# npit/video-learning-tf

Hardware: AMD Instinct MI355X
Metric: clips/sec (16-frame 227x227) LRCN train step (higher is better)
Workload: dtype f32; 1 GPU; LRCN AlexNet(fc6)+LSTM(256) 16-frame 227x227x3 clips, 101 classes, UCF-101-shaped synthetic, full train step; global_batch=64, clips_per_gpu=64, frames_per_clip=16, parallelism=dp1, optimizer=sgd+clip_by_global_norm(10), init=reference (sigma 0.05), dist_world_size=1

## Files before the change

video-learning-tf_amd/csrc/mfma_gemm.hip:

```cpp
#include <stdlib.h>
#include <string.h>

#include "common.h"
#include "conv_desc.h"

typedef float f32x16 __attribute__((ext_vector_type(16)));
typedef const __attribute__((address_space(4))) int* const_int_ptr;
__device__ __forceinline__ const_int_ptr as_const(const int* p) { return (const_int_ptr)(uintptr_t)p; }
static constexpr int NT = 256;
static constexpr int KBLK = 16;

static constexpr uint32_t OOB_OFF = 0xF0000000u;
static constexpr int64_t MAX_BUF_BYTES = 0xE0000000ll;

__device__ __forceinline__ __amdgpu_buffer_rsrc_t make_rsrc(const float* base, int64_t bytes) {
    return __builtin_amdgcn_make_buffer_rsrc(const_cast<float*>(base), 0, (int)(uint32_t)bytes, 0x00020000);
}
__device__ __forceinline__ float buf_load(__amdgpu_buffer_rsrc_t r, uint32_t voff, int soff) {
    return __builtin_bit_cast(float, __builtin_amdgcn_raw_buffer_load_b32(r, (int)voff, soff, 0));
}

template <int BX, int BR>
struct LdsTile {
    static constexpr int STR = BR + 2;
// ... 799 lines not shown
            static_for<0, NMS>([&](auto MI) __attribute__((always_inline)) {
                constexpr int m = decltype(MI)::value;
                constexpr int prod = m / (TM * TN), a = (m % (TM * TN)) / TN, b = m % TN;
                acc[a][b] = mfma_bf16(As[c][a].p[kProdA[prod]], Bs[c][b].p[kProdB[prod]], acc[a][b]);
                constexpr int idx = st * NMS + m;
                static_for<0, FPM>([&](auto EI) __attribute__((always_inline)) {
                    constexpr int f = idx * FPM + decltype(EI)::value;
                    if constexpr (f < NF) {
                        if constexpr (X4) dma_x4(cur ^ 1, f, rt_next);
                        else dma(cur ^ 1, f, rt_next);
                    }
                });
                __builtin_amdgcn_sched_barrier(0x106);
                if constexpr (idx == LT) load_table(rt_next + 1);
                if constexpr (idx == PIN) {
                    int rtn = rt_next + 1;
                    asm volatile("" : "+s"(rtn));
                    decode(rtn);
                    pin_table();
                }
            });
        });
        finish_tile(cur ^ 1);
    };
    auto run_tile = [&](const int cur, int rt_next) __attribute__((always_inline)) {
        if constexpr (MATH != 0) tile_split(cur, rt_next);
        else tile(cur, rt_next);
    };
    int rt = rt0;
    for (int i = 0; i + 1 < ntiles; i += 2, rt += 2) {
        run_tile(0, rt + 1);
        run_tile(1, rt + 2);
    }
    if (ntiles > 0 && (ntiles & 1)) run_tile(0, rt + 1);

    EpiRowMajor::template apply<TM, TN>(pe, zg, zs, i0 + wi0, j0 + wj0, acc);
    if (ones_row >= 0) {
        float* dbs = db_slabs + (int64_t)zs * db_stride + zg * d.Cog;
        const int lr = ones_row - wi0;
        if (lr >= 0 && lr < BM / WM) {
            const int a = lr >> 5, rr = lr & 31;
            const int q = (rr & 3) + 4 * (rr >> 3);
            if (((rr >> 2) & 1) == (lane >> 5)) {
#pragma unroll
                for (int b = 0; b < TN; ++b) {
                    const int j = j0 + wj0 + 32 * b + (lane & 31);
                    float v = 0.f;
#pragma unroll
                    for (int aa = 0; aa < TM; ++aa)
#pragma unroll
                        for (int qq = 0; qq < 16; ++qq)
                            if (aa == a && qq == q) v = acc[aa][b][qq];
                    if (j < d.Cog) dbs[j] = v;
                }
            }
        }
    }
}

typedef float f32x4 __attribute__((ext_vector_type(4)));
typedef float f32x4u __attribute__((ext_vector_type(4), aligned(4)));

struct ConvDmaParams {
    const float* w;
    int64_t w_ld;
    int64_t w_grp_stride;
    int64_t w_bytes;
    const int* row_tab;
    int nblk;
};

struct ConvRowClasses {
    int ncls;
    int wg0[6];
    int S[5];
    int oh0[5], RW[5];
    FastDiv dRW[5];
    int K[5], tab0[5], rt0[5];
};

struct ConvTile {
    int bid;
    int S, oh0, RW;
    FastDiv dRW;
    int K, nblk;
    const int* ktab;
    const int* row_tab;
};

__device__ __forceinline__ ConvTile conv_pick_tile(const ConvRowClasses& rc, const ConvGeom& g, const ConvDmaParams& pa) {
    const int id = blockIdx.x;
    int w0 = 0, w1 = rc.wg0[1], S = rc.S[0], oh0 = rc.oh0[0], RW = rc.RW[0], K = rc.K[0], tab0 = rc.tab0[0], rt0 = rc.rt0[0];
    FastDiv dRW = rc.dRW[0];
#pragma unroll
    for (int c = 1; c < 5; ++c) {
        if (c < rc.ncls && id >= rc.wg0[c]) {
            w0 = rc.wg0[c]; w1 = rc.wg0[c + 1]; S = rc.S[c]; oh0 = rc.oh0[c]; RW = rc.RW[c]; K = rc.K[c]; tab0 = rc.tab0[c]; rt0 = rc.rt0[c];
            dRW = rc.dRW[c];
        }
    }
    ConvTile t;
    t.bid = xcd_swizzle(id - w0, w1 - w0);
    t.S = S; t.oh0 = oh0; t.RW = RW; t.dRW = dRW; t.K = K; t.nblk = (K + KBLK - 1) / KBLK;
    t.ktab = g.ktab + tab0;
    t.row_tab = pa.row_tab + rt0;
    return t;
}

struct ConvPixel {
    uint32_t n, p, oh, ow;
};
__device__ __forceinline__ ConvPixel conv_tile_pixel(const ConvTile& t, uint32_t m, const FastDiv& dOW, int OW) {
    ConvPixel q;
    q.n = fd_div(m, t.dRW);
    q.p = m - q.n * t.RW;
    const uint32_t r = fd_div(q.p, dOW);
    q.ow = q.p - r * OW;
    q.oh = r + t.oh0;
    return q;
}

template <int BM>
__device__ __forceinline__ uint32_t conv_weight_voff(int i0, int cl, int Cog) {
    return (cl < BM && i0 + cl < Cog) ? (uint32_t)(i0 + cl) * 4u : OOB_OFF;
}
__device__ __forceinline__ uint32_t conv_pixel_voff(const ConvTile& tl, const ConvGeom& g, int m) {
    const bool vm = m < tl.S;
    const ConvPixel q = conv_tile_pixel(tl, vm ? m : 0, g.dOW, g.OW);
    const int ih0 = (int)q.oh * g.stride - g.pt + g.halo, iw0 = (int)q.ow * g.col_mul + g.col_add;
    return vm ? (uint32_t)((int64_t)q.n * g.img_stride + (int64_t)ih0 * g.Wp + iw0) * 4u : OOB_OFF;
}

template <int SR>
struct ConvStageTab {
    int tabv[SR / 4];
    int row0 = 0;
    bool blk_ok = false;
    __device__ __forceinline__ void load(const ConvTile& tl, const ConvGeom& g, int wrow, int st) {
        const int k0 = st * SR + wrow;
        const const_int_ptr tt = as_const(tl.ktab) + k0 + st * g.zero;
#pragma unroll
        for (int f = 0; f < SR / 4; ++f) tabv[f] = tt[f];
        row0 = as_const(tl.row_tab)[k0 / KBLK + st * g.zero] + k0 % KBLK;
        blk_ok = k0 / KBLK < tl.nblk;
    }
    __device__ __forceinline__ void pin() {
#pragma unroll
        for (int f = 0; f < SR / 4; ++f) asm volatile("" : "+s"(tabv[f]));
        asm volatile("" : "+s"(row0));
    }
};

template <int SR>
__global__ __launch_bounds__(NT, 64 / SR) void conv_dma_kernel(const ConvDmaParams pa, const ConvGeom g, const EpiConvNCHW::Params pe, const ConvRowClasses rc,
                                                               int tiles_i, int wide) {
    constexpr int BM = 128, BN = 128;
    constexpr int ABUF = SR * BM, BUF = SR * (BM + BN);
    constexpr int RW = SR / 4;
    constexpr int NF = RW * 4;
    constexpr int NT2 = SR / 4;
    constexpr int FPM = 1;
    static_assert(SR == 64 || SR == 32, "stage depth");
    extern __shared__ __attribute__((aligned(16))) float ldsc[];
    const ConvTile tl = conv_pick_tile(rc, g, pa);
    const int ti_blk = tl.bid % tiles_i, tj_blk = tl.bid / tiles_i;
    const int zg = blockIdx.y;
    const int i0 = ti_blk * BM, j0 = tj_blk * BN;
    const int lane = threadIdx.x & 63;
    const int wave = __builtin_amdgcn_readfirstlane(threadIdx.x >> 6);
    const int wm = wave >> 1, wn = wave & 1;

    const i32x4 rs_w = rsrc_words(pa.w + (int64_t)zg * pa.w_grp_stride, pa.w_bytes - (int64_t)zg * pa.w_grp_stride * 4);
    const i32x4 rs_x = rsrc_words(g.x + (int64_t)zg * g.grp_stride, (g.total - (int64_t)zg * g.grp_stride) * 4);
    uint32_t voff_a[2], voff_b[2];
#pragma unroll
    for (int hf = 0; hf < 2; ++hf) {
        voff_a[hf] = conv_weight_voff<BM>(i0, hf * 64 + lane, pe.Cog);
        voff_b[hf] = conv_pixel_voff(tl, g, j0 + hf * 64 + lane);
    }
    const uint32_t lds0 = (uint32_t)(uintptr_t)(__attribute__((address_space(3))) float*)ldsc;
    const int ld_bytes = (int)(pa.w_ld * 4);

    ConvStageTab<SR> tab;
    int (&tabv)[RW] = tab.tabv;
    int& row0 = tab.row0;
    bool& blk_ok = tab.blk_ok;
    const int wrow = wave * RW;
    auto load_table = [&](int st) { tab.load(tl, g, wrow, st); };
    auto pin_table = [&]() { tab.pin(); };
    auto dma = [&](const int nb, const int f, int st) {
        const int rr = f >> 2, kind = f & 3, hf = kind & 1;
        const int z = st * g.zero;
        const uint32_t row_lds = lds0 + (uint32_t)(nb * BUF + (wrow + rr) * 128 + hf * 64 + z) * 4u;
        const bool live = blk_ok && st * SR + wrow + rr < tl.K;
        if (kind < 2) lds_dma_row(rs_w, row_lds, voff_a[hf], min(row0 + rr, g.K - 1) * ld_bytes);
        else lds_dma_row(rs_x, row_lds + ABUF * 4u, live ? voff_b[hf] : OOB_OFF, tabv[rr]);
    };
    int a_soff = 0;
    auto dma_fast = [&](const int nb, const int f, int st) {
        const int rr = f >> 2, kind = f & 3, hf = kind & 1;
        const uint32_t row_lds = lds0 + (uint32_t)(nb * BUF + (wrow + rr) * 128 + hf * 64 + st * g.zero) * 4u;
        if (f == 0) a_soff = row0 * ld_bytes;
        if (kind < 2) lds_dma_row(rs_w, row_lds, voff_a[hf], a_soff);
        else lds_dma_row(rs_x, row_lds + ABUF * 4u, voff_b[hf], tabv[rr]);
        if (kind == 1) a_soff += ld_bytes;
    };
    auto finish_stage = [&]() {
        asm volatile("s_waitcnt vmcnt(0)" ::: "memory");
        __syncthreads();
    };

    f32x16 acc[2][2];
#pragma unroll
    for (int a = 0; a < 2; ++a)
#pragma unroll
        for (int b = 0; b < 2; ++b)
#pragma unroll
            for (int q = 0; q < 16; ++q) acc[a][b][q] = 0.f;

    const int nstages = (tl.nblk * KBLK + SR - 1) / SR;
    load_table(0);
    pin_table();
#pragma unroll
    for (int f = 0; f < NF; ++f) dma(0, f, 0);
    load_table(1);
    pin_table();
    finish_stage();

    float bias_r[2][16];
#pragma unroll
    for (int a = 0; a < 2; ++a)
#pragma unroll
        for (int q = 0; q < 16; ++q) {
            const int co = i0 + wm * 64 + 2 * ((q & 3) + 8 * (q >> 2) + 4 * (lane >> 5)) + a;
            bias_r[a][q] = (pe.bias && co < pe.Cog) ? pe.bias[zg * pe.Cog + co] : 0.f;
        }

    const float* fa = ldsc + (lane >> 5) * 128 + wm * 64 + 2 * (lane & 31);
    const float* fb = ldsc + ABUF + (lane >> 5) * 128 + wn * 64 + (lane & 31);

    auto stage = [&](const int cur, const bool fast, int st_next) {
        float2 af[2], bf[2], an[2], bn[2];
        auto read_b = [&](int step) {
            const float* q = fb + cur * BUF + step * 256;
            return float2{q[0], q[32]};
        };
        af[0] = *reinterpret_cast<const float2*>(fa + cur * BUF);
        bf[0] = read_b(0);
        af[1] = *reinterpret_cast<const float2*>(fa + cur * BUF + 256);
        bf[1] = read_b(1);
#pragma unroll
        for (int t = 0; t < NT2; ++t) {
            if (t + 1 < NT2) {
#pragma unroll
                for (int u = 0; u < 2; ++u) {
                    an[u] = *reinterpret_cast<const float2*>(fa + cur * BUF + (2 * (t + 1) + u) * 256);
                    bn[u] = read_b(2 * (t + 1) + u);
                }
            }
#pragma unroll
            for (int m = 0; m < 8; ++m) {
                const int u = m >> 2, a = (m >> 1) & 1, b = m & 1;
                acc[a][b] = __builtin_amdgcn_mfma_f32_32x32x2f32(a ? af[u].y : af[u].x, b ? bf[u].y : bf[u].x, acc[a][b], 0, 0, 0);
                const int f = (t * 8 + m) * FPM;
                if (f < NF) {
#pragma unroll
                    for (int e = 0; e < FPM; ++e) {
                        if (fast) dma_fast(cur ^ 1, f + e, st_next);
                        else dma(cur ^ 1, f + e, st_next);
                    }
                    __builtin_amdgcn_sched_barrier(0);
                }
            }
            static_assert(NF / FPM / 8 <= NT2 - 4, "fetches must end before the table is replaced");
            if (t == NT2 - 4) {
                load_table(st_next + 1);
                __builtin_amdgcn_sched_barrier(0);
            }
            if (t == NT2 - 2) {
                pin_table();
                __builtin_amdgcn_sched_barrier(0);
            }
#pragma unroll
            for (int u = 0; u < 2; ++u) {
                af[u] = an[u];
                bf[u] = bn[u];
            }
        }
        finish_stage();
    };
    const int nfull = tl.K / SR;
    int st = 0;
    for (; st + 2 < nfull; st += 2) {
        stage(0, true, st + 1);
        stage(1, true, st + 2);
    }
    for (; st < nstages; ++st) {
        if (st & 1) stage(1, false, st + 1);
        else stage(0, false, st + 1);
    }

    if (wide) {
        constexpr int SP = BN + 4;
        float* T = ldsc;
#pragma unroll
        for (int b = 0; b < 2; ++b)
#pragma unroll
            for (int a = 0; a < 2; ++a)
#pragma unroll
                for (int q = 0; q < 16; ++q) {
                    const int i = (q & 3) + 8 * (q >> 2) + 4 * (lane >> 5);
                    float v = acc[a][b][q] + bias_r[a][q];
                    if (pe.relu) v = fmaxf(v, 0.f);
                    T[(wm * 64 + 2 * i + a) * SP + wn * 64 + 32 * b + (lane & 31)] = v;
                }
        __syncthreads();
        const int px = 4 * (lane & 31);
        const int m = j0 + px;
        const uint32_t n = fd_div((uint32_t)min(m, tl.S - 1), tl.dRW);
        const int p = m - (int)n * tl.RW;
        const bool run4 = m + 3 < tl.S && p + 3 < tl.RW;
        const int64_t cbase = ((int64_t)n * pe.Cout_total + (int64_t)zg * pe.Cog) * pe.y_plane + tl.oh0 * pe.OW + p;
#pragma unroll
        for (int i = 0; i < BM / 8; ++i) {
            const int cl = wave * (BM / 4) + 2 * i + (lane >> 5);
            const int co = i0 + cl;
            const f32x4 v = *reinterpret_cast<const f32x4*>(T + cl * SP + px);
            if (co >= pe.Cog) continue;
            float* dst = pe.y + cbase + (int64_t)co * pe.y_plane;
            if (run4) {
                *reinterpret_cast<f32x4u*>(dst) = v;
            } else {
#pragma unroll
                for (int e = 0; e < 4; ++e) {
                    const int me = m + e;
                    if (me < tl.S) {
                        const uint32_t ne = fd_div((uint32_t)me, tl.dRW);
                        const int pe_ = me - (int)ne * tl.RW + tl.oh0 * pe.OW;
                        pe.y[((int64_t)ne * pe.Cout_total + (int64_t)zg * pe.Cog + co) * pe.y_plane + pe_] = v[e];
                    }
                }
            }
        }
        return;
    }
#pragma unroll
    for (int b = 0; b < 2; ++b) {
        const int m = j0 + wn * 64 + 32 * b + (lane & 31);
        if (m >= tl.S) continue;
        const ConvPixel px = conv_tile_pixel(tl, m, pe.dOW, pe.OW);
        const int64_t c0 = (int64_t)px.n * pe.Cout_total + (int64_t)zg * pe.Cog;
        const int64_t ybase = c0 * pe.y_plane + (int64_t)(px.oh + pe.y_halo) * pe.y_wp + px.ow + pe.y_halo;
        const int64_t mbase = c0 * pe.m_plane + (int64_t)(px.oh + pe.m_halo) * pe.m_wp + px.ow + pe.m_halo;
#pragma unroll
        for (int a = 0; a < 2; ++a) {
            float mk[16];
            if (pe.mask) {
#pragma unroll
                for (int q = 0; q < 16; ++q) {
                    const int co = i0 + wm * 64 + 2 * ((q & 3) + 8 * (q >> 2) + 4 * (lane >> 5)) + a;
                    mk[q] = co < pe.Cog ? pe.mask[mbase + (int64_t)co * pe.m_plane] : 0.f;
                }
            }
#pragma unroll
            for (int q = 0; q < 16; ++q) {
                const int i = (q & 3) + 8 * (q >> 2) + 4 * (lane >> 5);
                const int co = i0 + wm * 64 + 2 * i + a;
                if (co < pe.Cog) {
                    float v = acc[a][b][q] + bias_r[a][q];
                    if (pe.relu) v = fmaxf(v, 0.f);
                    if (pe.mask) v = mk[q] > 0.f ? v : 0.f;
                    pe.y[ybase + (int64_t)co * pe.y_plane] = v;
                }
            }
        }
    }
}


__global__ void conv_wsplit_kernel(const float* __restrict__ w, int64_t w_ld, int64_t w_grp_stride, const int* __restrict__ row_tab,
                                   int K, int Cog, int CogP, int nstages, int planes, uint32_t* __restrict__ out) {
    const int st = blockIdx.x, zg = blockIdx.y;
    const int row0 = row_tab[st];
    uint32_t* o = out + ((int64_t)zg * nstages + st) * planes * 8 * CogP;
    for (int idx = threadIdx.x; idx < 8 * CogP; idx += blockDim.x) {
        const int q = idx & 3, co = (idx >> 2) % CogP, h = idx / (4 * CogP);
        const int r = 8 * h + 2 * q, p = st * 16 + r;
        float x0 = 0.f, x1 = 0.f;
        if (co < Cog) {
            const float* src = w + (int64_t)(row0 + r) * w_ld + zg * w_grp_stride + co;
            if (p < K) x0 = src[0];
            if (p + 1 < K) x1 = src[w_ld];
        }
        int pc[3] = {0, 0, 0};
        split_pieces<3>(x0, x1, pc);
        for (int k = 0; k < planes; ++k) o[(int64_t)((2 * k + h) * CogP + co) * 4 + q] = (uint32_t)pc[k];
    }
}

struct ConvRingParams {
    const uint32_t* wsplit;
    int CogP;
    int nstages;
};

template <int MATH, int BM>
__global__ __launch_bounds__(512, 1) void conv_ring_kernel(const ConvRingParams pa, const ConvGeom g, const EpiConvNCHW::Params pe,
                                                           int tiles_i, int OWp, int Mp, FastDiv dOHWp, FastDiv dOWp) {
    constexpr int BN = BM == 128 ? 256 : 512, SR = 16, NBUF = BM == 128 ? 5 : 4;
    constexpr int NH = BN / 256;
    static_assert(BM == 128 || BM == 64, "channel tile");
    constexpr int NPL = MATH == 6 ? 3 : 2;
    constexpr int ABUF = NPL * 8 * BM, BUF = ABUF + SR * BN;
    constexpr int NAF = (NPL * 2 * (BM / 64) + 7) / 8;
    constexpr int FW = NAF + 2 * NH;
    constexpr int VMW = (NBUF - 3) * FW;
    constexpr int NP = split_products(MATH), NPC = split_pieces_of(MATH);
    constexpr int NM = (BM / 32) * (BN / 256) * NP;
    static_assert(SR == KBLK, "one stage = one block of the reduction order");
    extern __shared__ __attribute__((aligned(16))) float ldsr[];
    const int bid = xcd_swizzle(blockIdx.x, gridDim.x);
    const int ti_blk = bid % tiles_i, tj_blk = bid / tiles_i;
    const int zg = blockIdx.y;
    const int i0 = ti_blk * BM, j0 = tj_blk * BN;
    const int lane = threadIdx.x & 63;
    const int wave = __builtin_amdgcn_readfirstlane(threadIdx.x >> 6);
    constexpr int TA = BM / 32, TB = BN / 8 / 32, WPX = 32 * TB;
    const int OHWp = g.OHW / g.OW * OWp;
    const int nstages = pa.nstages;

    const int64_t stage_dw = (int64_t)NPL * 8 * pa.CogP;
    const uint32_t* wbase = pa.wsplit + (int64_t)zg * nstages * stage_dw;
    const i32x4 rs_w = rsrc_words(reinterpret_cast<const float*>(wbase), nstages * stage_dw * 4);
    constexpr int NPIECE = NPL * 2 * (BM / 64);
    int piece[NAF];
    uint32_t voff_a[NAF];
#pragma unroll
    for (int e = 0; e < NAF; ++e) {
        piece[e] = e == 0 ? wave % NPIECE : 8 + (wave & 3);
        voff_a[e] = BM == 128 ? (uint32_t)(((piece[e] >> 1) * pa.CogP + i0 + (piece[e] & 1) * 64 + lane) * 16)
                              : (uint32_t)((piece[e] * pa.CogP + i0 + lane) * 16);
    }
    const int stage_bytes = (int)(stage_dw * 4);
    const i32x4 rs_x = rsrc_words(g.x + (int64_t)zg * g.grp_stride, (g.total - (int64_t)zg * g.grp_stride) * 4);
    uint32_t voff_b[NH];
#pragma unroll
    for (int hf = 0; hf < NH; ++hf) {
        const int m = j0 + 256 * hf + 4 * lane;
        const bool vm = m < Mp;
        const uint32_t mm = vm ? m : 0;
        const uint32_t n = fd_div(mm, dOHWp);
        const uint32_t p = mm - n * OHWp;
        const uint32_t oh = fd_div(p, dOWp);
        const uint32_t ow = p - oh * OWp;
        const int ih0 = (int)oh * g.stride - g.pt + g.halo, iw0 = (int)ow * g.col_mul + g.col_add;
        voff_b[hf] = vm ? (uint32_t)((int64_t)n * g.img_stride + (int64_t)ih0 * g.Wp + iw0) * 4u : OOB_OFF;
    }
    const uint32_t lds0 = (uint32_t)(uintptr_t)(__attribute__((address_space(3))) float*)ldsr;

    int tab0 = 0, tab1 = 0;
    const int wrow = wave * 2;
    auto load_table = [&](int st) __attribute__((always_inline)) {
        const int sc = min(st, nstages - 1) + st * g.zero;
        const const_int_ptr tt = as_const(g.ktab) + sc * SR + wrow;
        tab0 = tt[0];
        tab1 = tt[1];
    };
    auto pin_table = [&]() __attribute__((always_inline)) {
        asm volatile("" : "+s"(tab0));
        asm volatile("" : "+s"(tab1));
    };
    auto dma = [&](const uint32_t wr, const int f, int st) __attribute__((always_inline)) {
        if (f < NAF) {
            lds_dma_row4(rs_w, lds0 + wr + (uint32_t)piece[f] * 1024u, voff_a[f], st * stage_bytes);
        } else {
            const int r = (f - NAF) / NH, hf = (f - NAF) % NH;
            const bool live = st * SR + wrow + r < g.K;
            lds_dma_row4(rs_x, lds0 + wr + (uint32_t)(ABUF + (wrow + r) * BN + 256 * hf) * 4u, live ? voff_b[hf] : OOB_OFF,
                         r == 0 ? tab0 : tab1);
        }
    };
    auto dma_fast = [&](const uint32_t wr, const int f, int st) __attribute__((always_inline)) {
        if (f < NAF) {
            lds_dma_row4(rs_w, lds0 + wr + (uint32_t)piece[f] * 1024u, voff_a[f], st * stage_bytes);
        } else {
            const int r = (f - NAF) / NH, hf = (f - NAF) % NH;
            lds_dma_row4(rs_x, lds0 + wr + (uint32_t)(ABUF + (wrow + r) * BN + 256 * hf) * 4u, voff_b[hf], r == 0 ? tab0 : tab1);
        }
    };

    f32x16 acc[TA][TB];
#pragma unroll
    for (int a = 0; a < TA; ++a)
#pragma unroll
        for (int b = 0; b < TB; ++b)
#pragma unroll
            for (int q = 0; q < 16; ++q) acc[a][b][q] = 0.f;

    const float* fa = ldsr + ((lane >> 5) * BM + (lane & 31)) * 4;
    const float* fb = ldsr + ABUF + (lane >> 5) * 8 * BN + wave * WPX + (lane & 31);
    struct Raw {
        float b[TB][8];
    };
    auto load_raw = [&](int rd, Raw& r) __attribute__((always_inline)) {
#pragma unroll
        for (int j = 0; j < 8; ++j) {
            const float* q = fb + rd + j * BN;
#pragma unroll
            for (int b = 0; b < TB; ++b) r.b[b][j] = q[32 * b];
        }
    };
    auto load_a = [&](int rd, SplitBf16 (&A)[TA]) __attribute__((always_inline)) {
#pragma unroll
        for (int a = 0; a < TA; ++a) {
#pragma unroll
            for (int k = 0; k < NPC; ++k) A[a].p[k] = *reinterpret_cast<const i32x4*>(fa + rd + k * 2 * BM * 4 + a * 32 * 4);
        }
    };
    auto split = [&](const Raw& r, SplitBf16 (&B)[TB]) __attribute__((always_inline)) {
#pragma unroll
        for (int j = 0; j < 4; ++j)
#pragma unroll
// ... 748 lines not shown
#pragma unroll
    for (int f = 0; f < NF; ++f) dma(0, f, 0);
    load_table(1);
    pin_table();
    finish_stage();

    const float* fa = ldsc + (lane >> 4) * SA + (lane & 15);
    const float* fb = ldsc + ABUF + (lane >> 4) * SB + wave * 32 + (lane & 15);

    auto stage = [&](const int cur, const bool fast, int st_next, const int nsteps) {
        float af[2][TA], bf[2][2];
        auto read = [&](int step, float (&a)[TA], float (&b)[2]) {
            const float* pa_ = fa + cur * BUF + step * 4 * SA;
            const float* pb_ = fb + cur * BUF + step * 4 * SB;
#pragma unroll
            for (int i = 0; i < TA; ++i) a[i] = pa_[16 * i];
#pragma unroll
            for (int i = 0; i < 2; ++i) b[i] = pb_[16 * i];
        };
        read(0, af[0], bf[0]);
#pragma unroll
        for (int t = 0; t < NSTEP; ++t) {
            const int c = t & 1;
            if (t + 1 < NSTEP) read(t + 1, af[c ^ 1], bf[c ^ 1]);
            if (t < nsteps) {
#pragma unroll
                for (int m = 0; m < NM; ++m) {
                    const int a = m >> 1, b = m & 1;
                    acc[a][b] = __builtin_amdgcn_mfma_f32_16x16x4f32(af[c][a], bf[c][b], acc[a][b], 0, 0, 0);
                    const int i = t * NM + m, f = i / FSP;
                    if (i % FSP == 0 && f < NF) {
                        if (fast) dma_fast(cur ^ 1, f, st_next);
                        else dma(cur ^ 1, f, st_next);
                        __builtin_amdgcn_sched_barrier(0);
                    }
                }
            } else {
#pragma unroll
                for (int m = 0; m < NM; ++m) {
                    const int i = t * NM + m, f = i / FSP;
                    if (i % FSP == 0 && f < NF) dma(cur ^ 1, f, st_next);
                }
            }
            if (t == LT) {
                load_table(st_next + 1);
                __builtin_amdgcn_sched_barrier(0);
            }
            if (t == NSTEP - 1) {
                pin_table();
                __builtin_amdgcn_sched_barrier(0);
            }
        }
        finish_stage();
    };
    const int nfull = tl.K / SR;
    const int last_steps = (tl.K - (nstages - 1) * SR + 3) / 4;
    int st = 0;
    for (; st + 2 < nfull; st += 2) {
        stage(0, true, st + 1, NSTEP);
        stage(1, true, st + 2, NSTEP);
    }
    for (; st < nstages; ++st) {
        const int ns = st == nstages - 1 ? last_steps : NSTEP;
        if (st & 1) stage(1, false, st + 1, ns);
        else stage(0, false, st + 1, ns);
    }

    if (wide) {
        constexpr int SP = BN + 4;
        float* T = ldsc;
#pragma unroll
        for (int b = 0; b < 2; ++b)
#pragma unroll
            for (int a = 0; a < TA; ++a)
#pragma unroll
                for (int q = 0; q < 4; ++q) {
                    float v = acc[a][b][q] + bias_r[a][q];
                    if (pe.relu) v = fmaxf(v, 0.f);
                    T[(16 * a + 4 * (lane >> 4) + q) * SP + wave * 32 + 16 * b + (lane & 15)] = v;
                }
        __syncthreads();
        const int px = 4 * (lane & 31);
        const int m = j0 + px;
        const uint32_t n = fd_div((uint32_t)min(m, tl.S - 1), tl.dRW);
        const int p = m - (int)n * tl.RW;
        const bool run4 = m + 3 < tl.S && p + 3 < tl.RW;
        const int64_t cbase = ((int64_t)n * pe.Cout_total + (int64_t)zg * pe.Cog) * pe.y_plane + tl.oh0 * pe.OW + p;
#pragma unroll
        for (int i = 0; i < BM / 8; ++i) {
            const int cl = wave * (BM / 4) + 2 * i + (lane >> 5);
            const int co = i0 + cl;
            const f32x4 v = *reinterpret_cast<const f32x4*>(T + cl * SP + px);
            if (co >= pe.Cog) continue;
            float* dst = pe.y + cbase + (int64_t)co * pe.y_plane;
            if (run4) {
                *reinterpret_cast<f32x4u*>(dst) = v;
            } else {
#pragma unroll
                for (int e = 0; e < 4; ++e) {
                    const int me = m + e;
                    if (me < tl.S) {
                        const uint32_t ne = fd_div((uint32_t)me, tl.dRW);
                        const int pe_ = me - (int)ne * tl.RW + tl.oh0 * pe.OW;
                        pe.y[((int64_t)ne * pe.Cout_total + (int64_t)zg * pe.Cog + co) * pe.y_plane + pe_] = v[e];
                    }
                }
            }
        }
        return;
    }
#pragma unroll
    for (int b = 0; b < 2; ++b) {
        const int m = j0 + wave * 32 + 16 * b + (lane & 15);
        if (m >= tl.S) continue;
        const ConvPixel px = conv_tile_pixel(tl, m, pe.dOW, pe.OW);
        const int64_t c0 = (int64_t)px.n * pe.Cout_total + (int64_t)zg * pe.Cog;
        const int64_t ybase = c0 * pe.y_plane + (int64_t)(px.oh + pe.y_halo) * pe.y_wp + px.ow + pe.y_halo;
        const int64_t mbase = c0 * pe.m_plane + (int64_t)(px.oh + pe.m_halo) * pe.m_wp + px.ow + pe.m_halo;
        float mk[TA][4];
        if (pe.mask) {
#pragma unroll
            for (int a = 0; a < TA; ++a)
#pragma unroll
                for (int q = 0; q < 4; ++q) {
                    const int co = i0 + 16 * a + 4 * (lane >> 4) + q;
                    mk[a][q] = co < pe.Cog ? pe.mask[mbase + (int64_t)co * pe.m_plane] : 0.f;
                }
        }
#pragma unroll
        for (int a = 0; a < TA; ++a) {
#pragma unroll
            for (int q = 0; q < 4; ++q) {
                const int co = i0 + 16 * a + 4 * (lane >> 4) + q;
                if (co < pe.Cog) {
                    float v = acc[a][b][q] + bias_r[a][q];
                    if (pe.relu) v = fmaxf(v, 0.f);
                    if (pe.mask) v = mk[a][q] > 0.f ? v : 0.f;
                    pe.y[ybase + (int64_t)co * pe.y_plane] = v;
                }
            }
        }
    }
}


constexpr size_t conv16_stage_bytes(int BM, int SR) { return (size_t)2 * SR * ((BM + 63) / 64 * 64 + 16 + 144) * sizeof(float); }
constexpr size_t conv16_staging_bytes(int BM) { return (size_t)BM * (128 + 4) * sizeof(float); }
constexpr size_t conv16_lds_bytes(int BM, int SR) {
    return conv16_stage_bytes(BM, SR) > conv16_staging_bytes(BM) ? conv16_stage_bytes(BM, SR) : conv16_staging_bytes(BM);
}
static_assert(3 * conv16_lds_bytes(96, 16) <= 163840 && 3 * conv16_lds_bytes(48, 16) <= 163840, "three 16-row workgroups per CU");
static_assert(2 * conv16_lds_bytes(96, 32) <= 163840 && 2 * conv16_lds_bytes(48, 32) <= 163840, "two 32-row workgroups per CU");

template <int BM, int SR>
static int launch_conv_dma_sr(const ConvGeom& g, const float* w, int64_t w_ld, int w_grp_stride, const int* row_tab, int Cog,
                              int Cout_total, const ConvOut& o, hipStream_t s, const vl_conv_rowcls* rcd) {
    constexpr int BN = 128;
    static_assert(BM != 128 || SR == 32, "the 32x32 kernel launches with 32-row stages");
    constexpr size_t lds = BM == 128 ? (size_t)BM * (BN + 4) * sizeof(float) : conv16_lds_bytes(BM, SR);
    static_assert(BM != 128 || (size_t)2 * SR * (BM + BN) * sizeof(float) <= (size_t)BM * (BN + 4) * sizeof(float), "stage buffers fit");
    static_assert(BM == 128 || conv16_stage_bytes(BM, SR) <= lds, "stage buffers fit");
    ConvDmaParams pa{w, w_ld, (int64_t)w_grp_stride, (int64_t)g.K * w_ld * 4, row_tab, ceil_div(g.K, KBLK)};
    const EpiConvNCHW::Params pe = make_epi(g, Cog, Cout_total, o);
    static bool attr_set = false;
    if (!attr_set) {
        const void* kern;
        if constexpr (BM == 128) kern = reinterpret_cast<const void*>(conv_dma_kernel<SR>);
        else kern = reinterpret_cast<const void*>(conv_dma16_kernel<BM / 16, SR, SR == 16 ? 3 : 2>);
        VL_HIP(hipFuncSetAttribute(kern, hipFuncAttributeMaxDynamicSharedMemorySize, (int)lds));
        attr_set = true;
    }
    const int tiles_i = ceil_div(Cog, BM);
    ConvRowClasses rc;
    memset(&rc, 0, sizeof(rc));
    if (rcd && rcd->ncls > 1 && g_conv_row_classes) {
        const int nimg = g.M / g.OHW;
        rc.ncls = rcd->ncls;
        for (int c = 0; c < rc.ncls; ++c) {
            rc.RW[c] = rcd->rows[c] * g.OW; rc.dRW[c] = make_fastdiv(rc.RW[c]); rc.S[c] = nimg * rc.RW[c];
            rc.oh0[c] = rcd->oh0[c]; rc.K[c] = rcd->K[c]; rc.tab0[c] = rcd->tab0[c]; rc.rt0[c] = rcd->rt0[c];
            rc.wg0[c + 1] = rc.wg0[c] + tiles_i * ceil_div(rc.S[c], BN);
        }
    } else {
        rc.ncls = 1;
        rc.RW[0] = g.OHW; rc.dRW[0] = g.dOHW; rc.S[0] = g.M; rc.K[0] = g.K;
        rc.wg0[1] = tiles_i * ceil_div(g.M, BN);
    }
    dim3 grid(rc.wg0[rc.ncls], (unsigned)(Cout_total / Cog), 1);
    const int wide = (o.y_halo == 0 && !o.mask && !kConvNoWideStore && (size_t)BM * (BN + 4) * sizeof(float) <= lds) ? 1 : 0;
    if constexpr (BM == 128) {
        hipLaunchKernelGGL(conv_dma_kernel<SR>, grid, dim3(NT), lds, s, pa, g, pe, rc, tiles_i, wide);
    } else {
        hipLaunchKernelGGL((conv_dma16_kernel<BM / 16, SR, SR == 16 ? 3 : 2>), grid, dim3(NT), lds, s, pa, g, pe, rc, tiles_i, wide);
    }
    VL_LAUNCH_CHECK();
    g_conv_last_launch = BM * 100 + SR;
    return 0;
}

static int conv16_stage_depth(bool few) { return g_conv_stage_depth ? g_conv_stage_depth : few ? 32 : 16; }

template <int BM>
static int launch_conv_dma(const ConvGeom& g, const float* w, int64_t w_ld, int w_grp_stride, const int* row_tab, int Cog,
                           int Cout_total, const ConvOut& o, hipStream_t s, const vl_conv_rowcls* rcd = nullptr, bool few = false) {
    if constexpr (BM != 128) {
        if (conv16_stage_depth(few) == 16)
            return launch_conv_dma_sr<BM, 16>(g, w, w_ld, w_grp_stride, row_tab, Cog, Cout_total, o, s, rcd);
    }
    return launch_conv_dma_sr<BM, 32>(g, w, w_ld, w_grp_stride, row_tab, Cog, Cout_total, o, s, rcd);
}

template <int BM>
static int launch_conv_ring(const ConvGeom& g, const float* w, int64_t w_ld, int w_grp_stride, const int* row_tab, int Cog,
                            int Cout_total, const ConvOut& o, uint32_t* wsplit, hipStream_t s) {
    constexpr int BN = BM == 128 ? 256 : 512;
    const int math = g_conv_math, planes = math == 6 ? 3 : 2;
    const int groups = Cout_total / Cog, nstages = ceil_div(g.K, KBLK), CogP = ceil_div(Cog, BM) * BM;
    hipLaunchKernelGGL(conv_wsplit_kernel, dim3(nstages, groups), dim3(256), 0, s, w, w_ld, (int64_t)w_grp_stride, row_tab, g.K, Cog,
                       CogP, nstages, planes, wsplit);
    VL_LAUNCH_CHECK();
    ConvRingParams pa{wsplit, CogP, nstages};
    const EpiConvNCHW::Params pe = make_epi(g, Cog, Cout_total, o);
    const int OH = g.OHW / g.OW, OWp = (g.OW + 3) / 4 * 4, Mp = g.M / g.OW * OWp;
    const int tiles_i = ceil_div(Cog, BM), tiles_j = ceil_div(Mp, BN);
    dim3 grid(tiles_i * tiles_j, (unsigned)groups, 1);
    if (BM == 128 && math != 6 && !kRing8) {
        constexpr size_t lds4 = (size_t)3 * 16 * (128 + 256) * sizeof(float);
        static bool attr4[2] = {false, false};
        const int v4 = math == 3;
        auto k4 = v4 ? conv_ring4_kernel<3> : conv_ring4_kernel<1>;
        if (!attr4[v4]) {
            VL_HIP(hipFuncSetAttribute(reinterpret_cast<const void*>(k4), hipFuncAttributeMaxDynamicSharedMemorySize, (int)lds4));
            attr4[v4] = true;
        }
        hipLaunchKernelGGL(k4, grid, dim3(256), lds4, s, pa, g, pe, tiles_i, OWp, Mp, make_fastdiv(OH * OWp), make_fastdiv(OWp));
        VL_LAUNCH_CHECK();
        return 0;
    }
    const size_t lds = (size_t)(BM == 128 ? 5 : 4) * (planes * 8 * BM + 16 * BN) * sizeof(float);
    static bool attr_set[3] = {false, false, false};
    const int v8 = math == 6 ? 2 : math == 3 ? 1 : 0;
    auto kern = v8 == 2 ? conv_ring_kernel<6, BM> : v8 == 1 ? conv_ring_kernel<3, BM> : conv_ring_kernel<1, BM>;
    if (!attr_set[v8]) {
        VL_HIP(hipFuncSetAttribute(reinterpret_cast<const void*>(kern), hipFuncAttributeMaxDynamicSharedMemorySize, (int)lds));
        attr_set[v8] = true;
    }
    hipLaunchKernelGGL(kern, grid, dim3(512), lds, s, pa, g, pe, tiles_i, OWp, Mp, make_fastdiv(OH * OWp), make_fastdiv(OWp));
    VL_LAUNCH_CHECK();
    return 0;
}

template <bool PADDED>
static int dispatch_conv(const ConvGeom& g, const float* w, int64_t w_ld, int w_grp_stride, const int* row_tab, int Cog,
                         int Cout_total, const ConvOut& o, uint32_t* wsplit, hipStream_t s, const vl_conv_rowcls* rcd) {
    g_conv_last_launch = 0;
    const int w128 = ceil_div(Cog, 128) * 128, w96 = ceil_div(Cog, 96) * 96, w64 = ceil_div(Cog, 64) * 64;
    if (g_conv_math != 0 && PADDED && g.col_mul == 1 && wsplit != nullptr) {
        if (Cog >= 96) return launch_conv_ring<128>(g, w, w_ld, w_grp_stride, row_tab, Cog, Cout_total, o, wsplit, s);
        if (Cog >= 40 && Cog <= 64) return launch_conv_ring<64>(g, w, w_ld, w_grp_stride, row_tab, Cog, Cout_total, o, wsplit, s);
    }
    const bool dma_ok = PADDED && (int64_t)g.K * w_ld * 4 < MAX_BUF_BYTES && !kConvStaged;
    const int64_t px = ceil_div(g.M, 128), cus = vl_device_cus(), ngrp = Cout_total / Cog;
    const bool few = px * ceil_div(Cog, 128) * ngrp < 8 * cus;
    if (dma_ok && few && !kConvNoLoadPick) {
        const int widths[3] = {128, 96, 48};
        auto pick = [&](int64_t pxt, int64_t& load) {
            int b = 0;
            for (int i = 0; i < 3; ++i) {
                const int64_t l = ceil_div(pxt * ceil_div(Cog, widths[i]) * ngrp, cus) * widths[i];
                if (i == 0 || l < load) { b = i; load = l; }
            }
            return b;
        };
        auto run = [&](int wi, const ConvGeom& gg, const ConvOut& oo) {
            if (wi == 0) return launch_conv_dma<128>(gg, w, w_ld, w_grp_stride, row_tab, Cog, Cout_total, oo, s, nullptr, true);
            if (wi == 1) return launch_conv_dma<96>(gg, w, w_ld, w_grp_stride, row_tab, Cog, Cout_total, oo, s, nullptr, true);
            return launch_conv_dma<48>(gg, w, w_ld, w_grp_stride, row_tab, Cog, Cout_total, oo, s, nullptr, true);
        };
        int64_t best_load = 0;
        const int best = pick(px, best_load);
        const int nimg = g.M / g.OHW;
        const int64_t wgs_per_px = (int64_t)ceil_div(Cog, widths[best]) * ngrp;
        const int64_t rounds = px * wgs_per_px / cus;
        if (rounds >= 6 && !kConvNoTailSplit) {
            const int64_t px_a = rounds * cus / wgs_per_px;
            const int n_a = (int)(px_a * 128 / g.OHW);
            const int n_b = nimg - n_a;
            if (n_a > 0 && n_b > 0) {
                int64_t load_b = 0;
                const int64_t px_b = ceil_div((int64_t)n_b * g.OHW, 128);
                const int wb = pick(px_b, load_b);
                const int64_t load_a = ceil_div(ceil_div((int64_t)n_a * g.OHW, 128) * wgs_per_px, cus) * widths[best];
                if ((load_a + (load_b > 64 ? load_b : 64) + 16) * 100 <= best_load * 95) {
                    ConvGeom ga = g, gb = g;
                    ga.M = n_a * g.OHW; ga.total = g.img_stride * n_a;
                    gb.x = g.x + (int64_t)n_a * g.img_stride; gb.M = n_b * g.OHW; gb.total = g.img_stride * n_b;
                    ConvOut ob = o;
                    ob.y = o.y + (int64_t)n_a * Cout_total * (o.OH + 2 * o.y_halo) * (o.OW + 2 * o.y_halo);
                    if (o.mask) ob.mask = o.mask + (int64_t)n_a * Cout_total * (o.OH + 2 * o.m_halo) * (o.OW + 2 * o.m_halo);
                    if (int rc = run(best, ga, o)) return rc;
                    return run(wb, gb, ob);
                }
            }
        }
        return run(best, g, o);
    }
    if (w128 <= w96 && w128 <= w64) {
        if (dma_ok) {
            return launch_conv_dma<128>(g, w, w_ld, w_grp_stride, row_tab, Cog, Cout_total, o, s, rcd);
        }
        return launch_conv<128, 2, 2, PADDED>(g, w, w_ld, w_grp_stride, row_tab, Cog, Cout_total, o, s);
    }
    if (dma_ok && ceil_div(Cog, 48) * 48 < w64 && ceil_div(Cog, 48) * 48 < w96)
        return launch_conv_dma<48>(g, w, w_ld, w_grp_stride, row_tab, Cog, Cout_total, o, s, rcd);
    if (w96 <= w64) {
        if (dma_ok)
            return launch_conv_dma<96>(g, w, w_ld, w_grp_stride, row_tab, Cog, Cout_total, o, s, rcd);
        return launch_conv<96, 1, 4, PADDED>(g, w, w_ld, w_grp_stride, row_tab, Cog, Cout_total, o, s);
    }
    return launch_conv<64, 1, 4, PADDED>(g, w, w_ld, w_grp_stride, row_tab, Cog, Cout_total, o, s);
}

static void fill_geom(ConvGeom& g, const float* x, int n, int cin_total, int cig, int H, int W, int halo, int OH, int OW,
                      int stride, int pt, int pl, int K, const int* tab, const int2* tab2, int phase = 1) {
    g.x = x; g.ktab = tab; g.ktab2 = tab2; g.K = K; g.M = n * OH * OW; g.H = H; g.W = W;
    g.halo = halo;
    g.Wp = phase > 1 ? (W + 2 * halo + phase - 1) / phase : W + 2 * halo;
    g.col_mul = phase > 1 ? 1 : stride;
    g.col_add = phase > 1 ? 0 : halo - pl;
    g.stride = stride; g.pt = pt; g.pl = pl; g.OHW = OH * OW; g.OW = OW;
    g.dOHW = make_fastdiv(g.OHW); g.dOW = make_fastdiv(g.OW);
    const int64_t Pp = (int64_t)(H + 2 * halo) * g.Wp;
    g.img_stride = (int64_t)cin_total * phase * Pp;
    g.grp_stride = (int64_t)cig * phase * Pp;
    g.total = g.img_stride * n;
    g.zero = 0;
}

extern "C" int vl_conv_fwd(const vl_conv_desc* d, const float* x, const float* w, const float* bias, float* y, int n,
                           int relu, vl_stream_t stream) {
    VL_CHECK(d && x && w && y, "vl_conv_fwd: null argument");
    VL_CHECK(n > 0 && (int64_t)n * d->oh * d->ow < (1ll << 31), "vl_conv_fwd: bad batch %d", n);
    ConvGeom g;
    fill_geom(g, x, n, d->cin, d->cig, d->h, d->w, d->x_halo, d->oh, d->ow, d->stride, d->pt, d->pl, d->K, d->ptab_fwd, d->ptab2_fwd,
              d->x_phase > 1 ? d->x_phase : 1);
    VL_CHECK(g.total * 4 < MAX_BUF_BYTES, "vl_conv_fwd: input of %lld elements exceeds the buffer-offset range", (long long)g.total);
    ConvOut o{y, bias, nullptr, relu, d->y_halo, 0, d->oh, d->ow};
    if (d->fwd_padded) return dispatch_conv<true>(g, w, d->cout, d->cog, d->rowtab_fwd, d->cog, d->cout, o, d->wsplit_fwd, (hipStream_t)stream, &d->rc_fwd);
    return dispatch_conv<false>(g, w, d->cout, d->cog, d->rowtab_fwd, d->cog, d->cout, o, d->wsplit_fwd, (hipStream_t)stream, &d->rc_fwd);
}

__global__ __launch_bounds__(256) void conv_wt_transpose_kernel(const float* __restrict__ w, float* __restrict__ wt, int KH, int KW,
                                                                int cig, int cog, int groups) {
    __shared__ float tile[64][65];
    const int cin = cig * groups, cout = cog * groups;
    const int tci = (cig + 63) / 64, tco = (cog + 63) / 64;
    int b = blockIdx.x;
    const int co0 = (b % tco) * 64; b /= tco;
    const int ci0 = (b % tci) * 64; b /= tci;
    const int g = b % groups;       b /= groups;
    const int kx = b % KW, ky = b / KW;
// ... 457 lines not shown
```

Measured before the change: 1928 clips/s.

## Add 16-row stage depth to 128x128 conv kernel for three workgroups per CU

The 128x128 direct-DMA conv kernel gains a 16-row K-stage variant (SR=16), now chosen by default unless few tiles are present. It shrinks LDS per workgroup so three workgroups fit per CU, and launch bounds request three. To make that fit, the wide-store epilogue is split into two half-tile passes, and bias loading moves after the main loop so it does not hold registers during the K loop. The last stage skips prefetch. Shallower stages mean more barriers per K, and two-pass stores add a sync.

```diff
diff --git a/video-learning-tf_amd/csrc/mfma_gemm.hip b/video-learning-tf_amd/csrc/mfma_gemm.hip
--- a/video-learning-tf_amd/csrc/mfma_gemm.hip
+++ b/video-learning-tf_amd/csrc/mfma_gemm.hip
@@ -975,7 +975,7 @@
 };
 
 template <int SR>
-__global__ __launch_bounds__(NT, 64 / SR) void conv_dma_kernel(const ConvDmaParams pa, const ConvGeom g, const EpiConvNCHW::Params pe, const ConvRowClasses rc,
+__global__ __launch_bounds__(NT, SR == 16 ? 3 : 64 / SR) void conv_dma_kernel(const ConvDmaParams pa, const ConvGeom g, const EpiConvNCHW::Params pe, const ConvRowClasses rc,
                                                                int tiles_i, int wide) {
     constexpr int BM = 128, BN = 128;
     constexpr int ABUF = SR * BM, BUF = SR * (BM + BN);
@@ -983,7 +983,12 @@
     constexpr int NF = RW * 4;
     constexpr int NT2 = SR / 4;
     constexpr int FPM = 1;
-    static_assert(SR == 64 || SR == 32, "stage depth");
+    constexpr int FLAST = (NF - 1) / FPM / 8;
+    constexpr int LT = FLAST > NT2 - 4 ? FLAST : NT2 - 4;
+    constexpr int PT = SR == 16 ? NT2 - 1 : NT2 - 2;
+    static_assert(SR == 64 || SR == 32 || SR == 16, "stage depth");
+    static_assert(SR % KBLK == 0 && KBLK % RW == 0, "a wave's rows lie within one 16-row block");
+    static_assert(NF / FPM <= 8 * NT2 && FLAST <= LT && LT <= PT && PT <= NT2 - 1, "fetches must end before the table is replaced");
     extern __shared__ __attribute__((aligned(16))) float ldsc[];
     const ConvTile tl = conv_pick_tile(rc, g, pa);
     const int ti_blk = tl.bid % tiles_i, tj_blk = tl.bid / tiles_i;
@@ -1051,18 +1056,20 @@
     finish_stage();
 
     float bias_r[2][16];
-#pragma unroll
-    for (int a = 0; a < 2; ++a)
-#pragma unroll
-        for (int q = 0; q < 16; ++q) {
-            const int co = i0 + wm * 64 + 2 * ((q & 3) + 8 * (q >> 2) + 4 * (lane >> 5)) + a;
-            bias_r[a][q] = (pe.bias && co < pe.Cog) ? pe.bias[zg * pe.Cog + co] : 0.f;
-        }
+    if constexpr (SR != 16) {
+#pragma unroll
+        for (int a = 0; a < 2; ++a)
+#pragma unroll
+            for (int q = 0; q < 16; ++q) {
+                const int co = i0 + wm * 64 + 2 * ((q & 3) + 8 * (q >> 2) + 4 * (lane >> 5)) + a;
+                bias_r[a][q] = (pe.bias && co < pe.Cog) ? pe.bias[zg * pe.Cog + co] : 0.f;
+            }
+    }
 
     const float* fa = ldsc + (lane >> 5) * 128 + wm * 64 + 2 * (lane & 31);
     const float* fb = ldsc + ABUF + (lane >> 5) * 128 + wn * 64 + (lane & 31);
 
-    auto stage = [&](const int cur, const bool fast, int st_next) {
+    auto stage = [&](const int cur, const bool fast, int st_next, const bool fetch = true) {
         float2 af[2], bf[2], an[2], bn[2];
         auto read_b = [&](int step) {
             const float* q = fb + cur * BUF + step * 256;
@@ -1086,7 +1093,7 @@
                 const int u = m >> 2, a = (m >> 1) & 1, b = m & 1;
                 acc[a][b] = __builtin_amdgcn_mfma_f32_32x32x2f32(a ? af[u].y : af[u].x, b ? bf[u].y : bf[u].x, acc[a][b], 0, 0, 0);
                 const int f = (t * 8 + m) * FPM;
-                if (f < NF) {
+                if (fetch && f < NF) {
 #pragma unroll
                     for (int e = 0; e < FPM; ++e) {
                         if (fast) dma_fast(cur ^ 1, f + e, st_next);
@@ -1095,12 +1102,11 @@
                     __builtin_amdgcn_sched_barrier(0);
                 }
             }
-            static_assert(NF / FPM / 8 <= NT2 - 4, "fetches must end before the table is replaced");
-            if (t == NT2 - 4) {
+            if (fetch && t == LT) {
                 load_table(st_next + 1);
                 __builtin_amdgcn_sched_barrier(0);
             }
-            if (t == NT2 - 2) {
+            if (fetch && t == PT) {
                 pin_table();
                 __builtin_amdgcn_sched_barrier(0);
             }
@@ -1118,12 +1124,30 @@
         stage(0, true, st + 1);
         stage(1, true, st + 2);
     }
-    for (; st < nstages; ++st) {
+    const int ntail = SR == 16 ? nstages - 1 : nstages;
+    for (; st < ntail; ++st) {
         if (st & 1) stage(1, false, st + 1);
         else stage(0, false, st + 1);
     }
-
-    if (wide) {
+    if constexpr (SR == 16) {
+        if (st & 1) stage(1, false, st + 1, false);
+        else stage(0, false, st + 1, false);
+#pragma unroll
+        for (int a = 0; a < 2; ++a)
+#pragma unroll
+            for (int q = 0; q < 16; ++q) {
+                const int co = i0 + wm * 64 + 2 * ((q & 3) + 8 * (q >> 2) + 4 * (lane >> 5)) + a;
+                bias_r[a][q] = (pe.bias && co < pe.Cog) ? pe.bias[zg * pe.Cog + co] : 0.f;
+            }
+#pragma unroll
+        for (int a = 0; a < 2; ++a)
+#pragma unroll
+            for (int b = 0; b < 2; ++b)
+#pragma unroll
+                for (int q = 0; q < 16; ++q) acc[a][b][q] += bias_r[a][q];
+    }
+
+    if (SR != 16 && wide) {
         constexpr int SP = BN + 4;
         float* T = ldsc;
 #pragma unroll
@@ -1167,6 +1191,57 @@
         }
         return;
     }
+    if (SR == 16 && wide) {
+        constexpr int SP = BN + 4;
+        float* T = ldsc;
+        constexpr int NPASS = 2, PR = BM / NPASS;
+        const int px = 4 * (lane & 31);
+        const int m = j0 + px;
+        const uint32_t n = fd_div((uint32_t)min(m, tl.S - 1), tl.dRW);
+        const int p = m - (int)n * tl.RW;
+        const bool run4 = m + 3 < tl.S && p + 3 < tl.RW;
+        const int64_t cbase = ((int64_t)n * pe.Cout_total + (int64_t)zg * pe.Cog) * pe.y_plane + tl.oh0 * pe.OW + p;
+#pragma unroll
+        for (int ps = 0; ps < NPASS; ++ps) {
+            if (ps) __syncthreads();
+            if (wm == ps) {
+#pragma unroll
+                for (int b = 0; b < 2; ++b)
+#pragma unroll
+                    for (int a = 0; a < 2; ++a)
+#pragma unroll
+                        for (int q = 0; q < 16; ++q) {
+                            const int i = (q & 3) + 8 * (q >> 2) + 4 * (lane >> 5);
+                            float v = acc[a][b][q];
+                            if (pe.relu) v = fmaxf(v, 0.f);
+                            T[(2 * i + a) * SP + wn * 64 + 32 * b + (lane & 31)] = v;
+                        }
+            }
+            __syncthreads();
+#pragma unroll
+            for (int i = 0; i < PR / 8; ++i) {
+                const int cl = wave * (PR / 4) + 2 * i + (lane >> 5);
+                const int co = i0 + ps * PR + cl;
+                const f32x4 v = *reinterpret_cast<const f32x4*>(T + cl * SP + px);
+                if (co >= pe.Cog) continue;
+                float* dst = pe.y + cbase + (int64_t)co * pe.y_plane;
+                if (run4) {
+                    *reinterpret_cast<f32x4u*>(dst) = v;
+                } else {
+#pragma unroll
+                    for (int e = 0; e < 4; ++e) {
+                        const int me = m + e;
+                        if (me < tl.S) {
+                            const uint32_t ne = fd_div((uint32_t)me, tl.dRW);
+                            const int pe_ = me - (int)ne * tl.RW + tl.oh0 * pe.OW;
+                            pe.y[((int64_t)ne * pe.Cout_total + (int64_t)zg * pe.Cog + co) * pe.y_plane + pe_] = v[e];
+                        }
+                    }
+                }
+            }
+        }
+        return;
+    }
 #pragma unroll
     for (int b = 0; b < 2; ++b) {
         const int m = j0 + wn * 64 + 32 * b + (lane & 31);
@@ -1190,7 +1265,7 @@
                 const int i = (q & 3) + 8 * (q >> 2) + 4 * (lane >> 5);
                 const int co = i0 + wm * 64 + 2 * i + a;
                 if (co < pe.Cog) {
-                    float v = acc[a][b][q] + bias_r[a][q];
+                    float v = SR == 16 ? acc[a][b][q] : acc[a][b][q] + bias_r[a][q];
                     if (pe.relu) v = fmaxf(v, 0.f);
                     if (pe.mask) v = mk[q] > 0.f ? v : 0.f;
                     pe.y[ybase + (int64_t)co * pe.y_plane] = v;
@@ -2245,14 +2320,21 @@
 static_assert(3 * conv16_lds_bytes(96, 16) <= 163840 && 3 * conv16_lds_bytes(48, 16) <= 163840, "three 16-row workgroups per CU");
 static_assert(2 * conv16_lds_bytes(96, 32) <= 163840 && 2 * conv16_lds_bytes(48, 32) <= 163840, "two 32-row workgroups per CU");
 
+constexpr size_t conv128_stage_bytes(int SR) { return (size_t)2 * SR * (128 + 128) * sizeof(float); }
+constexpr size_t conv128_pass_bytes(int SR) { return (size_t)(SR == 16 ? 64 : 128) * (128 + 4) * sizeof(float); }
+constexpr size_t conv128_lds_bytes(int SR, bool wide) {
+    return (wide || SR != 16) && conv128_pass_bytes(SR) > conv128_stage_bytes(SR) ? conv128_pass_bytes(SR) : conv128_stage_bytes(SR);
+}
+static_assert(3 * conv128_lds_bytes(16, true) <= 163840 && 3 * conv128_lds_bytes(16, false) <= 163840, "three 16-row workgroups per CU");
+static_assert(2 * conv128_lds_bytes(32, true) <= 163840 && 2 * conv128_lds_bytes(32, false) <= 163840, "two 32-row workgroups per CU");
+
 template <int BM, int SR>
 static int launch_conv_dma_sr(const ConvGeom& g, const float* w, int64_t w_ld, int w_grp_stride, const int* row_tab, int Cog,
                               int Cout_total, const ConvOut& o, hipStream_t s, const vl_conv_rowcls* rcd) {
     constexpr int BN = 128;
-    static_assert(BM != 128 || SR == 32, "the 32x32 kernel launches with 32-row stages");
-    constexpr size_t lds = BM == 128 ? (size_t)BM * (BN + 4) * sizeof(float) : conv16_lds_bytes(BM, SR);
-    static_assert(BM != 128 || (size_t)2 * SR * (BM + BN) * sizeof(float) <= (size_t)BM * (BN + 4) * sizeof(float), "stage buffers fit");
-    static_assert(BM == 128 || conv16_stage_bytes(BM, SR) <= lds, "stage buffers fit");
+    constexpr size_t lds_max = BM == 128 ? conv128_lds_bytes(SR, true) : conv16_lds_bytes(BM, SR);
+    static_assert(BM != 128 || conv128_stage_bytes(SR) <= conv128_lds_bytes(SR, false), "stage buffers fit");
+    static_assert(BM == 128 || conv16_stage_bytes(BM, SR) <= lds_max, "stage buffers fit");
     ConvDmaParams pa{w, w_ld, (int64_t)w_grp_stride, (int64_t)g.K * w_ld * 4, row_tab, ceil_div(g.K, KBLK)};
     const EpiConvNCHW::Params pe = make_epi(g, Cog, Cout_total, o);
     static bool attr_set = false;
@@ -2260,7 +2342,7 @@
         const void* kern;
         if constexpr (BM == 128) kern = reinterpret_cast<const void*>(conv_dma_kernel<SR>);
         else kern = reinterpret_cast<const void*>(conv_dma16_kernel<BM / 16, SR, SR == 16 ? 3 : 2>);
-        VL_HIP(hipFuncSetAttribute(kern, hipFuncAttributeMaxDynamicSharedMemorySize, (int)lds));
+        VL_HIP(hipFuncSetAttribute(kern, hipFuncAttributeMaxDynamicSharedMemorySize, (int)lds_max));
         attr_set = true;
     }
     const int tiles_i = ceil_div(Cog, BM);
@@ -2280,7 +2362,9 @@
         rc.wg0[1] = tiles_i * ceil_div(g.M, BN);
     }
     dim3 grid(rc.wg0[rc.ncls], (unsigned)(Cout_total / Cog), 1);
-    const int wide = (o.y_halo == 0 && !o.mask && !kConvNoWideStore && (size_t)BM * (BN + 4) * sizeof(float) <= lds) ? 1 : 0;
+    const int wide = (o.y_halo == 0 && !o.mask && !kConvNoWideStore &&
+                      (BM == 128 || (size_t)BM * (BN + 4) * sizeof(float) <= lds_max)) ? 1 : 0;
+    const size_t lds = BM == 128 ? conv128_lds_bytes(SR, wide != 0) : lds_max;
     if constexpr (BM == 128) {
         hipLaunchKernelGGL(conv_dma_kernel<SR>, grid, dim3(NT), lds, s, pa, g, pe, rc, tiles_i, wide);
     } else {
@@ -2293,13 +2377,16 @@
 
 static int conv16_stage_depth(bool few) { return g_conv_stage_depth ? g_conv_stage_depth : few ? 32 : 16; }
 
+static int conv128_stage_depth(bool few) { return g_conv_stage_depth ? g_conv_stage_depth : few ? 32 : 16; }
+
+template <int BM>
+static int conv_stage_depth(bool few) { return BM == 128 ? conv128_stage_depth(few) : conv16_stage_depth(few); }
+
 template <int BM>
 static int launch_conv_dma(const ConvGeom& g, const float* w, int64_t w_ld, int w_grp_stride, const int* row_tab, int Cog,
                            int Cout_total, const ConvOut& o, hipStream_t s, const vl_conv_rowcls* rcd = nullptr, bool few = false) {
-    if constexpr (BM != 128) {
-        if (conv16_stage_depth(few) == 16)
-            return launch_conv_dma_sr<BM, 16>(g, w, w_ld, w_grp_stride, row_tab, Cog, Cout_total, o, s, rcd);
-    }
+    if (conv_stage_depth<BM>(few) == 16)
+        return launch_conv_dma_sr<BM, 16>(g, w, w_ld, w_grp_stride, row_tab, Cog, Cout_total, o, s, rcd);
     return launch_conv_dma_sr<BM, 32>(g, w, w_ld, w_grp_stride, row_tab, Cog, Cout_total, o, s, rcd);
 }
 
```

After: 1934 clips/s, median of 6. About the same (+0.3%).
